# cwfparsonson/ddls

Hardware: NVIDIA H100
Metric: env_steps_per_sec (higher is better)
Workload: dtype f64

## Files before the change

ddls_b200/csrc/ramp_engine.cu:

```cuda
#include <algorithm>
#include <cmath>
#include <cstdio>
#include <cstdlib>
#include <cstring>
#include <map>
#include <mutex>
#include <numeric>
#include <utility>
#include <vector>

#include "ramp_kernels.cuh"
#include "ramp_env.cuh"
#include "ramp_owned.cuh"

using namespace ramp;

namespace {

constexpr int MAX_EVENT_PAIRS = 64;
constexpr int RAMP_SMEM_CARVEOUT = 100;

using LookaheadKernel = void (*)(const LookaheadArgs);
constexpr int WARP_NT = 128, SPLIT_WARP_NT = 32;
LookaheadKernel warp_kernel() { return ramp_lookahead_kernel<WARP_NT / 32>; }
// ... 16 lines not shown
}

using StepKernel = void (*)(const StepArgs);
constexpr size_t STEP_SMEM_MAX = 200 * 1024;
StepKernel step_kernel_for(int nt) { return nt == 32 ? ramp_step_kernel<32> : ramp_step_kernel<1>; }

struct HostTemplate {
    TemplateDev dev;
    DeviceArray<unsigned char> blob;
    std::vector<unsigned char> bytes;
    uint64_t hash = 0;
    DeviceArray<unsigned char> res_blob;
};

struct ResultArrays {
    DeviceArray<double> jct, comm, comp, util;
    DeviceArray<int32_t> n_ticks, status, util_nmw;
    DeviceArray<int64_t> trace_off;
    cudaError_t alloc(size_t n) { return alloc_each(n, jct, comm, comp, util, n_ticks, status, util_nmw, trace_off); }
    ResultSlots view() const { return {jct.get(), comm.get(), comp.get(), n_ticks.get(), status.get(), trace_off.get(), util.get(), util_nmw.get()}; }
};

struct TraceArrays {
    DeviceArray<int32_t> n_active;
    DeviceArray<double> tick;
    DeviceArray<unsigned long long> top;
    cudaError_t alloc(uint64_t len) {
        const cudaError_t err = alloc_each(len, n_active, tick);
        return err == cudaSuccess ? top.alloc(1) : err;
    }
    TracePool view() const { return TracePool{n_active.get(), tick.get(), top.get(), (uint64_t)n_active.size()}; }
};

constexpr int N_WINDOWS = 4;
struct LookaheadWindow {
    Stream stream;
    Event ev_planned, ev_end, ev_consumed;
    DeviceArray<Counters> counters;
    DeviceArray<WorkItem> items_res, chunk_items;
    DeviceArray<ChunkDesc> chunks;
    DeviceArray<int32_t> rank, tcount, tbase;
    DeviceArray<SpecRecord> rec;
    DeviceArray<unsigned char> scratch;
};

}

struct ramp_engine {
    ramp_config_t cfg{};
    int sm_count = 0;
    Stream stream;
    std::vector<HostTemplate> templates;
    DeviceArray<TemplateDev> d_templates;
    uint64_t max_scratch = 0;
    int32_t max_w = 1, max_c = 1;
    int32_t par_cap = 0;
    uint32_t memo_cap = 0;
    DeviceArray<unsigned long long> d_memo_keys;
    DeviceArray<int32_t> d_memo_vals;
    DeviceArray<unsigned long long> d_memo_keys2;
    uint32_t memo_cap2 = 0;
    ResultArrays res;
    int32_t n_slots = 0;
    TraceArrays pool;
    DeviceArray<WorkItem> d_items;
    DeviceArray<Counters> d_counters;
    DeviceArray<MemoStats> d_stats;
    DeviceArray<ramp_action_t> d_actions;
    DeviceArray<double> d_step_stats;
    DeviceArray<int32_t> d_n_cluster_steps;
    DeviceArray<double> d_ep_export;
    DeviceArray<double> d_es_export;
    EpisodeState ep{};
    DeviceArray<double> ep_ef, ep_es, ep_rf, tick_util; DeviceArray<int32_t> ep_ei, ep_ri, tick_util_n; DeviceArray<ramp_job_record_t> ep_rec;
    DeviceArray<ramp_arrival_t> d_arrivals;
    DeviceArray<int32_t> d_n_jobs_ep;
    PinnedArray<ramp_arrival_t> h_arr_stage;
    Event ev_stage;
    int step_nt = 0;
    size_t step_smem = 0;
    DeviceArray<unsigned char> d_scratch;
    uint64_t scratch_stride = 0;
    int grid = 0;
    size_t smem_bytes = 0;
    int cta_nt = 0;
    int dense_grid = 0;
    size_t dense_smem_bytes = 0;
    double dense_factor = 2.0;
    int cta_grid = 0;
    int cta64_grid = 0;
    int cta256_grid = 0;
    int cta_grid_for(int nt) const { return nt == 256 ? cta256_grid : nt == 128 ? cta_grid : cta64_grid; }
    size_t cta_smem_bytes = 0;
    size_t smem2_bytes = 0;
    int debug = 0;
    int mode = 0;
    PinnedArray<int32_t> h_n_work;
    PinnedArray<MemoStats> h_stats;
    DeviceArray<WorkItem> d_items_big;
    Stream stream2;
    Event ev_fork, ev_join;
    int use_quotient = 1;
    int n_resident = 0, n_nonresident = 0;
    int32_t res_tmpl_cap = 0, res_n_cap = 0, res_spill_ops = 0, res_spill_deps = 0;
    int res_grid = 0;
    size_t res_smem = 0;
    DeviceArray<unsigned char> d_res_scratch;
    uint64_t res_scratch_stride = 0;
    DeviceArray<WorkItem> d_items_res;
    DeviceArray<WorkItem> d_chunk_items;
    DeviceArray<ChunkDesc> d_chunks;
    DeviceArray<int32_t> d_tcount;
    DeviceArray<int32_t> d_tbase;
    DeviceArray<int32_t> d_rank;
    DeviceArray<TemplateHints> d_hints;
    DeviceArray<double> d_hint_jct;
    bool has_env = false;
    EnvDev env{};
    std::vector<DeviceArray<unsigned char>> env_allocs;
    PinnedArray<int32_t> env_h_need;
    PinnedArray<unsigned char> env_h_mirror;
    bool env_unchecked_decide = false;
    bool env_agents_set = false;
    DeviceArray<double> steplog_stats, steplog_rewards;
    DeviceArray<int32_t> steplog_actions;
    DeviceArray<WorkItem> sa_chunk_items;
    DeviceArray<ChunkDesc> sa_chunks;
    ResultArrays sa_res;
    int32_t sa_cap = 0;
    DeviceArray<WorkItem> sa_items;
    DeviceArray<int32_t> sa_rank;
    DeviceArray<Counters> sa_counters;
    int overlap = 1;
    LookaheadWindow win[N_WINDOWS];
    bool win_ready = false;
    uint64_t win_seq = 0;
    Stream plan_stream;
    Event ev_reset;
    bool reset_pending = false;
    DeviceArray<unsigned long long> d_spec_keys, d_repair_keys;
// ... 200 lines not shown
    if (!src.empty()) memcpy(blob.data() + h.off_src, src.data(), sizeof(int32_t) * src.size());
    return true;
}

int identity_quotient(const ramp_lowered_job_t* j, ramp_quotient_t* q) {
    memset(q, 0, sizeof(*q));
    const int32_t N = j->n_ops, E = j->n_deps;
    std::vector<uint32_t> ok, dk;
    make_rank_keys(j->op_prio, N, ok);
    make_rank_keys(j->dep_prio, E, dk);
    q->n_ops = N; q->n_deps = E; q->n_workers = j->n_workers; q->n_channels = j->n_channels;
    q->op_cost = (double*)malloc(sizeof(double) * N); q->op_key = (uint32_t*)malloc(4 * (size_t)N); q->op_worker = (uint32_t*)malloc(4 * (size_t)N);
    q->op_weight = (uint32_t*)malloc(4 * (size_t)N); q->op_threshold = (uint32_t*)malloc(4 * (size_t)N); q->row_ptr = (int32_t*)malloc(4 * ((size_t)N + 1));
    const size_t e1 = std::max(E, 1);
    q->dep_dst = (int32_t*)malloc(4 * e1); q->dep_run_time = (double*)malloc(8 * e1); q->dep_key = (uint32_t*)malloc(4 * e1);
    q->dep_channel = (uint32_t*)malloc(4 * e1); q->dep_is_flow = (uint8_t*)malloc(e1); q->dep_inc = (uint32_t*)malloc(4 * e1);
    q->dep_group_mask = (uint64_t*)malloc(8 * e1); q->merged = 0; q->masks_valid = j->n_channels <= 64 ? 1 : 0;
    q->op_class = (int32_t*)malloc(4 * (size_t)N); q->dep_entry = (int32_t*)malloc(4 * e1);
    for (int32_t i = 0; i < N; ++i) {
        q->op_cost[i] = j->op_cost[i]; q->op_key[i] = ok[i]; q->op_worker[i] = j->op_worker[i]; q->op_weight[i] = 1;
        q->op_threshold[i] = j->op_n_parents[i]; q->row_ptr[i] = j->row_ptr[i]; q->op_class[i] = i;
    }
    q->row_ptr[N] = j->row_ptr[N];
    for (int32_t k = 0; k < E; ++k) {
        q->dep_dst[k] = j->dep_dst[k]; q->dep_run_time[k] = j->dep_run_time[k]; q->dep_key[k] = dk[k];
        q->dep_channel[k] = (j->dep_channel[k] == RAMP_NO_CHANNEL) ? 0xFFFFFFFFu : (uint32_t)j->dep_channel[k];
        q->dep_group_mask[k] = (j->dep_channel[k] == RAMP_NO_CHANNEL || !q->masks_valid) ? 0ull : (1ull << j->dep_channel[k]);
        q->dep_is_flow[k] = j->dep_is_flow[k] ? 1 : 0; q->dep_inc[k] = 1; q->dep_entry[k] = k;
    }
    return RAMP_OK;
}

int ensure_thread_scratch(ramp_engine* e) {
    const size_t smem = thread_smem_bytes(e->res_tmpl_cap, e->res_n_cap);
    if (smem > 220 * 1024) return set_error(RAMP_ERR_CAPACITY, "resident templates need %zu B of shared memory (max 220 KiB)", smem);
    if (smem != e->res_smem || e->res_grid == 0) {
        CUDA_TRY(reserve_dynamic_smem((const void*)ramp_lookahead_thread_kernel, smem));
        CUDA_TRY(cudaFuncSetAttribute(ramp_lookahead_thread_kernel, cudaFuncAttributePreferredSharedMemoryCarveout, RAMP_SMEM_CARVEOUT));
        int occ = 0;
        CUDA_TRY(cudaOccupancyMaxActiveBlocksPerMultiprocessor(&occ, ramp_lookahead_thread_kernel, RAMP_THREAD_CTA, smem));
        if (occ < 1) occ = 1;
        const int want = (e->cfg.n_episodes + 31) / 32 + 8;
        e->res_grid = std::max(1, std::min(std::min(e->sm_count * occ, e->sm_count * 2), want));
        e->res_smem = smem;
        if (e->debug) fprintf(stderr, "[ramp] thread kernel: %zu B dynamic shared memory, %d CTAs of %d threads per SM fit, grid %d\n",
                              smem, occ, RAMP_THREAD_CTA, e->res_grid);
    }
    const uint64_t stride = thread_scratch_bytes(e->res_spill_ops, e->res_spill_deps, e->cfg.trace_cap);
    if (stride != e->res_scratch_stride || stride * (uint64_t)e->res_grid != e->d_res_scratch.size()) {
        CUDA_TRY(cudaStreamSynchronize(e->stream.get()));
        CUDA_TRY(e->d_res_scratch.alloc(stride * (uint64_t)e->res_grid));
        e->res_scratch_stride = stride;
    }
    return RAMP_OK;
}

ThreadArgs make_thread_args(ramp_engine* e, const ChunkDesc* chunks, const WorkItem* chunk_items, Counters* c,
                            const ResultSlots& res, const TracePool& pool, MemoStats* stats) {
    ThreadArgs a{};
    a.templates = e->d_templates.get(); a.chunks = chunks; a.n_chunks = &c->n_chunks; a.cursor = &c->chunk_cursor; a.items = chunk_items;
    a.scratch = e->d_res_scratch.get(); a.scratch_stride = e->res_scratch_stride;
    a.res = res; a.pool = pool; a.trace_cap = e->cfg.trace_cap;
    a.tmpl_cap = e->res_tmpl_cap; a.n_cap = e->res_n_cap; a.spill_ops = e->res_spill_ops; a.spill_deps = e->res_spill_deps;
    a.stats = stats; a.hints = e->d_hints.get(); a.hint_jct = e->d_hint_jct.get();
    return a;
}

void bucket_resident(ramp_engine* e, const WorkItem* items, Counters* c, WorkItem* chunk_items, ChunkDesc* chunks, int32_t* rank,
                     int32_t* tcount, int32_t* tbase, cudaStream_t st) {
    BucketArgs ba{};
    ba.items = items; ba.n_items = &c->n_work_res; ba.n_templates = (int32_t)e->templates.size();
    ba.tcount = tcount; ba.tbase = tbase; ba.chunk_items = chunk_items; ba.chunks = chunks;
    ba.n_chunks = &c->n_chunks; ba.cursor = &c->chunk_cursor; ba.rank = rank;
    ramp_bucket_kernel<<<1, 1024, 0, st>>>(ba);
    e->launches++;
}

int launch_lookaheads(ramp_engine* e, const ChunkDesc* chunks, const WorkItem* chunk_items, int thread_grid,
                      const WorkItem* items, int n_small, const WorkItem* items_big, int n_big, Counters* c,
                      const ResultSlots& res, const TracePool& pool, MemoStats* stats, cudaStream_t st) {
    if (thread_grid > 0) {
        ThreadArgs ta = make_thread_args(e, chunks, chunk_items, c, res, pool, stats);
        ramp_lookahead_thread_kernel<<<thread_grid, RAMP_THREAD_CTA, e->res_smem, st>>>(ta);
        e->launches++;
    }
    if (n_small + n_big == 0) return RAMP_OK;
    LookaheadArgs a = make_lookahead_args(e, items, c, res, pool, stats);
    LookaheadArgs ab = a;
    ab.items = items_big; ab.n_work = &c->n_work_big; ab.cursor = &c->work_cursor_big;
    const int wpb = WARP_NT / 32;
    const int warp_slots = e->grid * wpb;
    const int reg_slots = e->cta_grid * 4;
    int split_nt = 0;
    if (e->mode != 1 && n_big > 0) {
// ... 52 lines not shown
    if (src && n) CUDA_TRY(cudaMemcpy(e->env_allocs.back().get(), src, sizeof(T) * n, cudaMemcpyHostToDevice));
    else CUDA_TRY(cudaMemset(e->env_allocs.back().get(), 0, sizeof(T) * std::max<size_t>(n, 1)));
    return RAMP_OK;
}

bool engine_owned(const ramp_engine* e, const void* p) {
    const uintptr_t q = (uintptr_t)p;
    auto in = [q](const void* base, size_t bytes) { return q >= (uintptr_t)base && q < (uintptr_t)base + bytes; };
    if (in(e->d_actions.get(), sizeof(ramp_action_t) * e->d_actions.size())) return true;
    for (const auto& a : e->env_allocs) if (in(a.get(), a.size())) return true;
    return false;
}

int ensure_windows(ramp_engine* e) {
    const int B = e->cfg.n_episodes;
    const size_t nt = (size_t)e->cfg.max_templates + 1;
    if (!e->win_ready) {
        CUDA_TRY(create(e->plan_stream, cudaStreamNonBlocking));
        CUDA_TRY(create(e->ev_reset, cudaEventDisableTiming));
        for (LookaheadWindow& w : e->win) {
            CUDA_TRY(create(w.stream, cudaStreamNonBlocking));
            CUDA_TRY(create(w.ev_planned, cudaEventDisableTiming));
            CUDA_TRY(create(w.ev_end, cudaEventDisableTiming));
            CUDA_TRY(create(w.ev_consumed, cudaEventDisableTiming));
            CUDA_TRY(w.counters.alloc(1));
            CUDA_TRY(cudaMemset(w.counters.get(), 0, sizeof(Counters)));
            CUDA_TRY(alloc_each(B, w.items_res, w.chunks, w.rank, w.rec));
            CUDA_TRY(w.chunk_items.alloc((size_t)B * 32));
            CUDA_TRY(alloc_each(nt, w.tcount, w.tbase));
            CUDA_TRY(cudaMemset(w.tcount.get(), 0, sizeof(int32_t) * nt));
        }
        e->win_ready = true;
    }
    const uint64_t bytes = e->res_scratch_stride * (uint64_t)e->res_grid;
    for (LookaheadWindow& w : e->win) {
        if (w.scratch.size() == bytes) continue;
        CUDA_TRY(cudaStreamSynchronize(e->stream.get()));
        CUDA_TRY(w.scratch.alloc(bytes));
    }
    return RAMP_OK;
}

void launch_step_kernel(ramp_engine* e, const ramp_action_t* d_actions, int32_t fuse, double* d_stats_out, int32_t* d_ncs_out) {
    const int B = e->cfg.n_episodes;
    StepArgs s{};
    s.actions = d_actions; s.ep = e->ep; s.res = e->res.view(); s.pool = e->pool.view(); s.counters = e->d_counters.get();
    s.stats_out = d_stats_out; s.n_cluster_steps_out = d_ncs_out; s.fuse_empty_steps = fuse;
    step_kernel_for(e->step_nt)<<<(B + e->step_nt - 1) / e->step_nt, e->step_nt, e->step_smem, e->stream.get()>>>(s);
    e->launches++;
}

int step_overlapped(ramp_engine* e, const ramp_action_t* d_actions, int32_t fuse, double* d_stats_out, int32_t* d_ncs_out) {
    int rc = ensure_windows(e);
    if (rc != RAMP_OK) return rc;
    const int B = e->cfg.n_episodes, grid_b = (B + 127) / 128;
    const int32_t n_templates = (int32_t)e->templates.size();
    LookaheadWindow& w = e->win[e->win_seq++ % N_WINDOWS];
    cudaStream_t ps = e->plan_stream.get(), ws = w.stream.get(), st = e->stream.get();
    if (e->ev_pending >= MAX_EVENT_PAIRS) { CUDA_TRY(cudaStreamSynchronize(st)); rc = resolve_events(e); if (rc) return rc; }
    CUDA_TRY(cudaStreamWaitEvent(ps, w.ev_consumed.get(), 0));
    if (e->reset_pending) { CUDA_TRY(cudaStreamWaitEvent(ps, e->ev_reset.get(), 0)); e->reset_pending = false; }
    SpecPlanArgs sp{};
    sp.actions = d_actions; sp.templates = e->d_templates.get(); sp.n_templates = n_templates; sp.B = B;
    sp.keys = e->d_spec_keys.get(); sp.mask = e->memo_cap - 1; sp.slot_base = e->spec_base;
    sp.items_res = w.items_res.get(); sp.counters = w.counters.get(); sp.rec = w.rec.get();
    ramp_spec_plan_kernel<<<grid_b, 128, 0, ps>>>(sp);
    CUDA_TRY(cudaEventRecord(e->ev_a[e->ev_pending].get(), ps));
    bucket_resident(e, w.items_res.get(), w.counters.get(), w.chunk_items.get(), w.chunks.get(), w.rank.get(), w.tcount.get(), w.tbase.get(), ps);
    CUDA_TRY(cudaEventRecord(w.ev_planned.get(), ps));
    CUDA_TRY(cudaStreamWaitEvent(ws, w.ev_planned.get(), 0));
    ThreadArgs ta = make_thread_args(e, w.chunks.get(), w.chunk_items.get(), w.counters.get(), e->res.view(), e->pool.view(), e->d_stats.get());
    ta.scratch = w.scratch.get();
    ramp_lookahead_thread_kernel<<<e->res_grid, RAMP_THREAD_CTA, e->res_smem, ws>>>(ta);
    CUDA_TRY(cudaEventRecord(e->ev_b[e->ev_pending].get(), ws));
    e->ev_pending++;
    CUDA_TRY(cudaEventRecord(w.ev_end.get(), ws));
    CUDA_TRY(cudaStreamWaitEvent(st, w.ev_end.get(), 0));
    CommitArgs c{};
    c.actions = d_actions; c.templates = e->d_templates.get(); c.n_templates = n_templates; c.ep = e->ep;
    c.memo.keys = e->d_memo_keys.get(); c.memo.mask = e->memo_cap - 1; c.memo.mode = e->cfg.memo_mode; c.memo.vals = e->d_memo_vals.get();
    c.rec = w.rec.get(); c.repair_keys = e->d_repair_keys.get(); c.repair_mask = e->memo_cap - 1; c.repair_base = e->repair_base;
    c.items_res = w.items_res.get(); c.win_counters = w.counters.get(); c.counters = e->d_counters.get(); c.stats = e->d_stats.get();
    ramp_commit_kernel<<<grid_b, 128, 0, st>>>(c);
    bucket_resident(e, w.items_res.get(), w.counters.get(), w.chunk_items.get(), w.chunks.get(), w.rank.get(), w.tcount.get(), w.tbase.get(), st);
    ramp_lookahead_thread_kernel<<<e->res_grid, RAMP_THREAD_CTA, e->res_smem, st>>>(ta);
    launch_step_kernel(e, d_actions, fuse, d_stats_out, d_ncs_out);
    CUDA_TRY(cudaEventRecord(w.ev_consumed.get(), st));
    e->launches += 4;
    CUDA_TRY(cudaGetLastError());
    return RAMP_OK;
}

}

int ramp_internal_set_error(int code, const char* msg) { g_last_error = msg; return code; }
cudaStream_t ramp_internal_stream(ramp_engine_t* e) { return e->stream.get(); }
int ramp_internal_device(ramp_engine_t* e) { return e->cfg.device; }
void ramp_internal_count_launches(ramp_engine_t* e, int n) { e->launches += n; }
int ramp_internal_env_returns(ramp_engine_t* e, const double** ret, const int32_t** n_decided) {
    if (!e || !e->has_env) return set_error(RAMP_ERR_BAD_ARG, "no environment");
    *ret = e->env.ret;
    *n_decided = e->env.n_decided;
    return RAMP_OK;
}

extern "C" {

const char* ramp_last_error(void) { return g_last_error.c_str(); }

#ifdef RAMP_TICK_CLOCKS
int ramp_debug_tick_clocks(unsigned long long* out, int reset) {
    static unsigned long long h[RAMP_TC_MAX_CTAS][RAMP_TC_SHAPES][RAMP_TC_PHASES + 1];
    CUDA_TRY(cudaDeviceSynchronize());
    CUDA_TRY(cudaMemcpyFromSymbol(h, ramp::ramp_tick_clocks, sizeof(h)));
    memset(out, 0, sizeof(h[0]));
    for (int b = 0; b < RAMP_TC_MAX_CTAS; ++b)
        for (int s = 0; s < RAMP_TC_SHAPES; ++s)
            for (int i = 0; i <= RAMP_TC_PHASES; ++i) out[s * (RAMP_TC_PHASES + 1) + i] += h[b][s][i];
// ... 5 lines not shown
int ramp_engine_create(const ramp_config_t* cfg_in, ramp_engine_t** out) {
    if (!cfg_in || !out) return set_error(RAMP_ERR_BAD_ARG, "null argument");
    ramp_config_t cfg = *cfg_in;
    if (cfg.n_episodes < 1 || cfg.max_jobs < 1 || cfg.n_cluster_workers < 1)
        return set_error(RAMP_ERR_BAD_ARG, "n_episodes, max_jobs and n_cluster_workers must be >= 1");
    if (cfg.max_running < 1) cfg.max_running = cfg.n_cluster_workers;
    if (cfg.max_templates < 1) cfg.max_templates = 1024;
    if (cfg.trace_cap < 1) cfg.trace_cap = 16384;
    if (cfg.job_queue_capacity < 0) cfg.job_queue_capacity = 10;
    if (cfg.machine_epsilon == 0.0) cfg.machine_epsilon = 1e-7;
    if (cfg.memo_capacity_log2 <= 0) {
        int lg = 10;
        while ((1ll << lg) < (long long)cfg.n_episodes * 16 && lg < 26) ++lg;
        cfg.memo_capacity_log2 = lg;
    }
    CUDA_TRY(cudaSetDevice(cfg.device));
    std::unique_ptr<ramp_engine> e(new ramp_engine());
    e->cfg = cfg;
    if (const char* v = getenv("RAMP_LOOKAHEAD_CTA_THREADS")) {
        const int nt = atoi(v);
        if (lookahead_cta_kernel_for(nt) == nullptr) return set_error(RAMP_ERR_BAD_ARG, "RAMP_LOOKAHEAD_CTA_THREADS must be 64, 128 or 256");
        e->cta_nt = nt;
    }
    if (const char* v = getenv("RAMP_LOOKAHEAD_MODE")) {
        e->mode = !strcmp(v, "warp") ? 1 : !strcmp(v, "cta") ? 2 : 0;
        if (!strcmp(v, "thread_unfolded")) e->use_quotient = 0;
    }
    if (const char* v = getenv("RAMP_DEBUG")) e->debug = atoi(v);
    if (const char* v = getenv("RAMP_STEP_OVERLAP")) e->overlap = atoi(v) != 0;
    if (const char* v = getenv("RAMP_DENSE_FACTOR")) e->dense_factor = atof(v);
    cudaDeviceProp prop{};
    CUDA_TRY(cudaGetDeviceProperties(&prop, cfg.device));
    e->sm_count = prop.multiProcessorCount;
    CUDA_TRY(create(e->stream, cudaStreamNonBlocking));
    const int B = cfg.n_episodes;

    CUDA_TRY(e->d_templates.alloc(cfg.max_templates));
    e->memo_cap = 1u << cfg.memo_capacity_log2;
    CUDA_TRY(e->d_memo_keys.alloc(e->memo_cap));
    CUDA_TRY(cudaMemset(e->d_memo_keys.get(), 0, sizeof(unsigned long long) * e->memo_cap));
    CUDA_TRY(e->d_memo_vals.alloc(e->memo_cap));
    e->memo_cap2 = 1;
    while (e->memo_cap2 < (uint32_t)cfg.max_templates * 2u) e->memo_cap2 <<= 1;
    CUDA_TRY(e->d_memo_keys2.alloc(e->memo_cap2));
    CUDA_TRY(cudaMemset(e->d_memo_keys2.get(), 0, sizeof(unsigned long long) * e->memo_cap2));
    e->spec_base = (int32_t)e->memo_cap + B + (int32_t)e->memo_cap2;
    e->repair_base = e->spec_base + (int32_t)e->memo_cap;
    e->n_slots = e->repair_base + (int32_t)e->memo_cap;
    CUDA_TRY(alloc_each(e->memo_cap, e->d_spec_keys, e->d_repair_keys));
    CUDA_TRY(cudaMemset(e->d_spec_keys.get(), 0, sizeof(unsigned long long) * e->memo_cap));
    CUDA_TRY(cudaMemset(e->d_repair_keys.get(), 0, sizeof(unsigned long long) * e->memo_cap));
    CUDA_TRY(e->res.alloc(e->n_slots));
    CUDA_TRY(cudaMemset(e->res.status.get(), 0, sizeof(int32_t) * e->n_slots));

    CUDA_TRY(e->pool.alloc(std::max<uint64_t>(4ull << 20, (uint64_t)B * 8ull * 2048ull)));
    CUDA_TRY(cudaMemset(e->pool.top.get(), 0, sizeof(unsigned long long)));

    CUDA_TRY(alloc_each(B, e->d_items, e->d_items_big, e->d_items_res, e->d_chunks, e->d_rank, e->d_actions, e->d_n_cluster_steps));
    CUDA_TRY(e->d_chunk_items.alloc((size_t)B * 32));
    CUDA_TRY(alloc_each((size_t)cfg.max_templates + 1, e->d_tcount, e->d_tbase));
    CUDA_TRY(cudaMemset(e->d_tcount.get(), 0, sizeof(int32_t) * ((size_t)cfg.max_templates + 1)));
    CUDA_TRY(e->d_hints.alloc(cfg.max_templates));
    CUDA_TRY(cudaMemset(e->d_hints.get(), 0, sizeof(TemplateHints) * (size_t)cfg.max_templates));
    CUDA_TRY(e->d_hint_jct.alloc(cfg.max_templates));
    CUDA_TRY(cudaMemset(e->d_hint_jct.get(), 0, sizeof(double) * (size_t)cfg.max_templates));
    CUDA_TRY(create(e->stream2, cudaStreamNonBlocking));
    CUDA_TRY(create(e->ev_fork, cudaEventDisableTiming));
// ... 148 lines not shown

    CUDA_TRY(cudaSetDevice(e->cfg.device));
    CUDA_TRY(ht.blob.alloc(total));
    CUDA_TRY(cudaMemcpy(ht.blob.get(), ht.bytes.data(), total, cudaMemcpyHostToDevice));
    unsigned char* base = ht.blob.get();
    TemplateDev& d = ht.dev;
    d.n_ops = N; d.n_deps = E; d.n_workers = W; d.n_channels = C;
    d.num_training_steps = j->num_training_steps; d.model_id = j->model_id; d.degree = j->degree;
    d.n_src = (int32_t)src.size(); d.canon_id = canon;
    d.size_class = ((int64_t)N + (int64_t)E >= BIG_THRESHOLD) ? 1 : 0;
    d.par_in_smem = par_in_smem ? 1 : 0;
    d._pad0 = 0;
    d.op_rec = (const int4*)(base + segs[0].off); d.op_n_parents = (const uint16_t*)(base + segs[1].off);
    d.op_row = (const int2*)(base + segs[2].off); d.dep_kd = (const unsigned long long*)(base + segs[3].off);
    d.dep_rt = (const double*)(base + segs[4].off); d.src_ops = (const int32_t*)(base + segs[5].off);
    d.kd_kmask = kd_kmask; d.kd_cmask = kd_cmask; d.kd_cshift = kd_cshift; d.kd_fshift = kd_fshift; d.kd_dshift = kd_dshift; d._pad1 = 0;
    d.scratch_bytes = scratch_bytes_for(N, E);
    d.algorithmic_bytes_static = 20ull * (uint64_t)N + 19ull * (uint64_t)E + 24ull;
    d.res_blob = nullptr; d.res_bytes = 0; d.res_n_ops = 0; d.res_n_deps = 0; d._pad2 = 0;
    if (e->mode == 0) {
        ramp_quotient_t q{};
        const int qrc = e->use_quotient ? ramp_quotient_template(j, &q) : identity_quotient(j, &q);
        if (qrc != RAMP_OK) return set_error(qrc, "ramp_quotient_template failed (%d)", qrc);
        std::vector<unsigned char> rblob;
        if (build_resident_blob(j, q, RESIDENT_MAX_BYTES, rblob)) {
            cudaError_t ce = ht.res_blob.alloc(rblob.size());
            if (ce == cudaSuccess) ce = cudaMemcpy(ht.res_blob.get(), rblob.data(), rblob.size(), cudaMemcpyHostToDevice);
            if (ce != cudaSuccess) { ramp_free_quotient(&q); return set_error(RAMP_ERR_CUDA, "resident blob upload failed: %s", cudaGetErrorString(ce)); }
            d.res_blob = ht.res_blob.get(); d.res_bytes = (int32_t)rblob.size();
            d.res_n_ops = q.n_ops; d.res_n_deps = q.n_deps;
            d.size_class = 2;
            e->res_tmpl_cap = std::max(e->res_tmpl_cap, (int32_t)align_up((uint64_t)rblob.size(), 128));
            e->res_n_cap = std::max(e->res_n_cap, (int32_t)align_up((uint64_t)q.n_ops, 2));
            e->res_spill_ops = std::max(e->res_spill_ops, q.n_ops);
            e->res_spill_deps = std::max(e->res_spill_deps, std::max(q.n_deps, 1));
        }
        if (e->debug) fprintf(stderr, "[ramp] template %d: N=%d E=%d W=%d C=%d -> quotient N=%d E=%d W=%d C=%d, %s (%zu B)\n", (int)e->templates.size(),
                              N, E, W, C, q.n_ops, q.n_deps, q.n_workers, q.n_channels, d.res_blob ? "resident" : "not resident", rblob.size());
        ramp_free_quotient(&q);
    }
    const int32_t id = (int32_t)e->templates.size();
    CUDA_TRY(cudaMemcpy(e->d_templates.get() + id, &d, sizeof(TemplateDev), cudaMemcpyHostToDevice));
    if (d.size_class == 2) e->n_resident++; else e->n_nonresident++;
    if (d.size_class != 2) {
        e->max_scratch = std::max(e->max_scratch, d.scratch_bytes);
        e->max_w = std::max(e->max_w, W);
        e->max_c = std::max(e->max_c, std::max(C, 1));
        if (d.par_in_smem) e->par_cap = std::max(e->par_cap, (int32_t)align_up((uint64_t)N, 16));
    }
    e->templates.push_back(std::move(ht));
    *id_out = id;
    return RAMP_OK;
}

int ramp_reset(ramp_engine_t* e, const ramp_arrival_t* arrivals, int32_t n_jobs) {
    if (!e || !arrivals) return set_error(RAMP_ERR_BAD_ARG, "null argument");
    if (n_jobs < 1 || n_jobs > e->cfg.max_jobs) return set_error(RAMP_ERR_BAD_ARG, "n_jobs %d not in [1, max_jobs=%d]", n_jobs, e->cfg.max_jobs);
    CUDA_TRY(cudaSetDevice(e->cfg.device));
    const int B = e->cfg.n_episodes;
    cudaStream_t st = e->stream.get();
    CUDA_TRY(cudaEventSynchronize(e->ev_stage.get()));
    const size_t row = sizeof(ramp_arrival_t) * (size_t)n_jobs;
    memcpy(e->h_arr_stage.get(), arrivals, row * B);
    if (n_jobs == e->cfg.max_jobs) {
        CUDA_TRY(cudaMemcpyAsync(e->d_arrivals.get(), e->h_arr_stage.get(), row * B, cudaMemcpyHostToDevice, st));
    } else {
// ... 733 lines not shown
```

ddls_b200/csrc/ramp_lookahead_thread.cuh:

```cuda
#pragma once

namespace ramp {

#ifndef RAMP_T_OCAP
#define RAMP_T_OCAP 8
#endif
#ifndef RAMP_T_FCAP
#define RAMP_T_FCAP 16
#endif
#ifndef RAMP_T_FASTF
#define RAMP_T_FASTF 6
#endif
#ifndef RAMP_T_NFCAP
#define RAMP_T_NFCAP 8
#endif
#define RAMP_T_WCAP 8
#define RAMP_T_CCAP 32
#ifndef RAMP_T_RING
#define RAMP_T_RING 32
#endif
#ifndef RAMP_T_PUB
#define RAMP_T_PUB 8
#endif
static_assert(RAMP_T_FCAP >= RAMP_T_FASTF && RAMP_T_OCAP >= 2 && RAMP_T_NFCAP >= 1, "shared-memory capacities below the small-frontier path");
#define RAMP_T_DONE 0x80000000u
#define RAMP_THREAD_CTA 64

struct ResHeader {
    int32_t n_ops, n_deps, n_workers, n_channels;
    int32_t n_src, num_training_steps, orig_workers, _pad0;
    uint32_t kmask, cmask, imask, _pad1;
    int32_t cshift, fshift, ishift, dshift;
    int32_t off_op_row, off_op_thr, off_out, off_src;
    int32_t total_bytes, _pad2, _pad3, _pad4;
};
static_assert(sizeof(ResHeader) == 96, "resident header is 96 bytes");

struct ChunkDesc { int32_t template_id, count; };
static_assert((RAMP_T_RING & (RAMP_T_RING - 1)) == 0 && (RAMP_T_PUB & (RAMP_T_PUB - 1)) == 0 && RAMP_T_PUB <= RAMP_T_RING,
              "ring and publish interval are powers of two");

struct __align__(16) TemplateHints { int32_t n_ticks, max_o, max_f, max_nf; };


struct ThreadArgs {
    const TemplateDev* templates;
    const ChunkDesc* chunks;
    const int32_t* n_chunks;
    int32_t* cursor;
    const WorkItem* items;
    unsigned char* scratch;
    uint64_t scratch_stride;
    ResultSlots res;
    TracePool pool;
    int32_t trace_cap;
    int32_t tmpl_cap;
    int32_t n_cap;
    int32_t spill_ops, spill_deps;
    MemoStats* stats;
    TemplateHints* hints;
    double* hint_jct;
};

__host__ __device__ inline size_t thread_smem_bytes(int tmpl_cap, int n_cap) {
    size_t per_lane = (size_t)RAMP_T_RING * 16 + (size_t)RAMP_T_FCAP * 16 + (size_t)RAMP_T_OCAP * 20 + (size_t)RAMP_T_NFCAP * 4
                      + (size_t)(RAMP_T_WCAP + RAMP_T_CCAP) * 4 + (size_t)n_cap * 2;
    return (size_t)tmpl_cap + 32 * per_lane + 64;
}
__host__ __device__ inline uint64_t thread_scratch_bytes(int spill_ops, int spill_deps, int trace_cap) {
    const uint64_t per_lane = (uint64_t)spill_ops * 20 + (uint64_t)spill_deps * 20 + (uint64_t)trace_cap * 12;
    return align_up(per_lane * 32, 256);
}

struct BucketArgs {
    const WorkItem* items;
    int32_t* n_items;
    int32_t n_templates;
    int32_t* tcount;
    int32_t* tbase;
    WorkItem* chunk_items;
    ChunkDesc* chunks;
    int32_t* n_chunks;
    int32_t* cursor;
    int32_t* rank;
};

__global__ void __launch_bounds__(1024) ramp_bucket_kernel(const BucketArgs a) {
    __shared__ int s_scan[1024];
    __shared__ int s_carry;
    const int n = *a.n_items;
    const int tid = threadIdx.x;
    for (int i = tid; i < n; i += blockDim.x) a.rank[i] = atomicAdd(&a.tcount[a.items[i].template_id], 1);
    if (tid == 0) s_carry = 0;
    __syncthreads();
    for (int base = 0; base < a.n_templates; base += blockDim.x) {
        const int t = base + tid;
        const int cnt = (t < a.n_templates) ? a.tcount[t] : 0;
        const int nch = (cnt + 31) >> 5;
        s_scan[tid] = nch;
// ... 463 lines not shown
        for (; k != end; ++k) {
            const int4 r = y.ring[(k & (RAMP_T_RING - 1)) * 32 + y.lane];
            const u64_t tick_b = rem_bits(r);
            const double tick = __longlong_as_double((long long)tick_b);
            const int n_active = r.z;
            if (r.w) S.comm = __dadd_rn(S.comm, tick);
            if (n_active > 0) {
                S.comp = __dadd_rn(S.comp, tick);
                if (do_util && tick_b != 0ull) {
                    if (n_active != util_last_n) { util_last_n = n_active; util_last_q = __ddiv_rn((double)n_active, y.util_dn); }
                    S.util = __dadd_rn(S.util, __dmul_rn(util_last_q, __ddiv_rn(tick, y.util_jct)));
                }
            }
            S.t = __dadd_rn(S.t, tick);
            if ((int)k < y.tr_cap) { y.tr_n[tr_idx] = n_active; y.tr_tick[tr_idx] = tick; tr_idx += y.tr_stride; }
#ifdef RAMP_T_LEDGER_NS
            __nanosleep(RAMP_T_LEDGER_NS);
#endif
        }
        st_release_cta(y.tail, k);
    }
    return S;
}

__global__ void __launch_bounds__(RAMP_THREAD_CTA) ramp_lookahead_thread_kernel(const ThreadArgs a) {
    extern __shared__ __align__(128) unsigned char smem_thr[];
    __shared__ __align__(8) unsigned long long mbar;
    __shared__ uint32_t s_head[32], s_tail[32];
    __shared__ SimFinal s_fin[32];
    __shared__ int32_t s_tr_cap[32];
    __shared__ int4 s_chunk;
    __shared__ int4 s_hint;
    __shared__ double s_hint_jct;
    const int lane = threadIdx.x & 31;
    const bool is_sim = threadIdx.x < 32;
    unsigned char* st = smem_thr + a.tmpl_cap;
    int4* ring = reinterpret_cast<int4*>(st);
    LaneCtx x;
    x.tm = smem_thr;
    x.f_sm = ring + RAMP_T_RING * 32;
    x.o_sm = x.f_sm + RAMP_T_FCAP * 32;
    x.nf_sm = reinterpret_cast<uint32_t*>(x.o_sm + RAMP_T_OCAP * 32);
    x.oi_sm = reinterpret_cast<int32_t*>(x.nf_sm + RAMP_T_NFCAP * 32);
    x.wk_sm = reinterpret_cast<uint32_t*>(x.oi_sm + RAMP_T_OCAP * 32);
    x.ck_sm = x.wk_sm + RAMP_T_WCAP * 32;
    x.cnt_sm = reinterpret_cast<uint16_t*>(x.ck_sm + RAMP_T_CCAP * 32);
    unsigned char* slab = a.scratch + (uint64_t)blockIdx.x * a.scratch_stride;
    x.f_gl = reinterpret_cast<int4*>(slab);
    x.o_gl = x.f_gl + (size_t)a.spill_deps * 32;
    double* tmp_tick = reinterpret_cast<double*>(x.o_gl + (size_t)a.spill_ops * 32);
    x.nf_gl = reinterpret_cast<uint32_t*>(tmp_tick + (size_t)a.trace_cap * 32);
    x.oi_gl = reinterpret_cast<int32_t*>(x.nf_gl + (size_t)a.spill_deps * 32);
    int32_t* tmp_n = x.oi_gl + (size_t)a.spill_ops * 32;
    x.ring = ring; x.head = &s_head[lane]; x.tail = &s_tail[lane]; x.fin = &s_fin[lane];
    x.lane = lane; x.n_cap = a.n_cap;

    if (threadIdx.x == 0) {
        asm volatile("mbarrier.init.shared::cta.b64 [%0], 1;" ::"r"(smem_u32(&mbar)));
        asm volatile("fence.mbarrier_init.release.cluster;" ::: "memory");
    }
    __syncthreads();
    uint32_t phase = 0;
    int loaded = -1;

    for (;;) {
        asm volatile("fence.proxy.async.shared::cta;" ::: "memory");
        if (threadIdx.x == 0) {
            int4 cd = make_int4(0, -1, 0, 0), hv = make_int4(0, 0, 0, 0);
            double hj = 0.0;
            const int c = atomicAdd(a.cursor, 1);
            if (c < *a.n_chunks) {
                const ChunkDesc ch = a.chunks[c];
                cd = make_int4(c, ch.template_id, ch.count, 0);
                const TemplateHints* hp = &a.hints[ch.template_id];
                int n_ticks = 0;
                asm volatile("ld.acquire.gpu.global.b32 %0, [%1];" : "=r"(n_ticks) : "l"(&hp->n_ticks) : "memory");
                if (n_ticks > 0) {
                    hv = make_int4(n_ticks, __ldcg(&hp->max_o), __ldcg(&hp->max_f), __ldcg(&hp->max_nf));
                    hj = __ldcg(&a.hint_jct[ch.template_id]);
                }
            }
            s_chunk = cd; s_hint = hv; s_hint_jct = hj;
        }
        __syncthreads();
        const int4 cd = s_chunk;
        if (cd.y < 0) break;
        const int c = cd.x, tmpl = cd.y, count = cd.z;
        TemplateHints hint;
        { const int4 hv = s_hint; hint.n_ticks = hv.x; hint.max_o = hv.y; hint.max_f = hv.z; hint.max_nf = hv.w; }
        const double hj = s_hint_jct;
        const TemplateDev& TD = a.templates[tmpl];
        if (tmpl != loaded) {
            if (threadIdx.x == 0) {
                const uint32_t bytes = (uint32_t)TD.res_bytes;
                asm volatile("mbarrier.arrive.expect_tx.shared::cta.b64 _, [%0], %1;" ::"r"(smem_u32(&mbar)), "r"(bytes) : "memory");
                asm volatile("cp.async.bulk.shared::cluster.global.mbarrier::complete_tx::bytes [%0], [%1], %2, [%3];"
                             ::"r"(smem_u32(smem_thr)), "l"(TD.res_blob), "r"(bytes), "r"(smem_u32(&mbar)) : "memory");
            }
            asm volatile(
                "{\n"
                ".reg .pred p;\n"
                "RAMP_WAIT_%=:\n"
                "mbarrier.try_wait.parity.shared::cta.b64 p, [%0], %1;\n"
                "@p bra RAMP_DONE_%=;\n"
                "bra RAMP_WAIT_%=;\n"
                "RAMP_DONE_%=:\n"
                "}\n" ::"r"(smem_u32(&mbar)), "r"(phase) : "memory");
            phase ^= 1u;
            loaded = tmpl;
        }
        const bool fast = hint.n_ticks > 0 && hint.n_ticks <= a.trace_cap && hint.max_o <= RAMP_T_OCAP && hint.max_f <= RAMP_T_FCAP
                          && hint.max_nf <= RAMP_T_NFCAP;
        const ResHeader& H = *reinterpret_cast<const ResHeader*>(x.tm);
        const bool active = lane < count;

        LedgerCtx y;
        WorkItem item;
        long long off = -1;
        int status0 = RAMP_ST_OK, nmw = 0, num_training_steps = 0, n_ops = 0, n_deps = 0;
        const bool direct = fast && a.pool.top != nullptr;
        if (!is_sim) {
            s_head[lane] = 0u; s_tail[lane] = 0u;
            if (active) {
                item = a.items[(size_t)c * 32 + lane];
                num_training_steps = H.num_training_steps; n_ops = H.n_ops; n_deps = H.n_deps;
                if (direct) {
                    const unsigned long long o = atomicAdd(a.pool.top, (unsigned long long)hint.n_ticks);
                    if (o + (unsigned long long)hint.n_ticks <= a.pool.len) off = (long long)o; else status0 = RAMP_ST_TRACE_OVERFLOW;
                }
                y.ring = ring; y.head = &s_head[lane]; y.tail = &s_tail[lane]; y.lane = lane;
                if (off >= 0) { y.tr_n = a.pool.n_active + off; y.tr_tick = a.pool.tick + off; y.tr_stride = 1; y.tr_cap = hint.n_ticks; }
                else { y.tr_n = tmp_n + lane; y.tr_tick = tmp_tick + lane; y.tr_stride = 32; y.tr_cap = a.trace_cap; }
                s_tr_cap[lane] = y.tr_cap;
                nmw = item.n_mounted_workers > 0 ? item.n_mounted_workers : H.orig_workers;
                y.util_jct = (fast && hj > 0.0 && !isinf(hj)) ? hj : 0.0;
                {
                    double dn = (double)nmw;
                    asm volatile("" : "+d"(dn));
                    y.util_dn = dn;
                }
            }
        }
        __syncthreads();

        if (is_sim) {
            if (active) {
                x.tr_cap = s_tr_cap[lane];
                if (fast) thread_lookahead<false>(x);
                else thread_lookahead<true>(x);
            }
            continue;
        }
        if (!active) continue;
        const LedgerSums S = ledger_run(y);
        const SimFinal R = s_fin[lane];
        int status = (R.status == RAMP_ST_OK) ? status0 : R.status;
        if (direct && status == RAMP_ST_OK && R.tick_no != hint.n_ticks) status = RAMP_ST_TRACE_OVERFLOW;
        if (!fast && status == RAMP_ST_OK) {
            TemplateHints* hp = &a.hints[tmpl];
            hp->max_o = R.max_o; hp->max_f = R.max_f; hp->max_nf = R.max_nf;
            a.hint_jct[tmpl] = __dmul_rn(S.t, (double)num_training_steps);
            asm volatile("st.release.gpu.global.b32 [%0], %1;" :: "l"(&hp->n_ticks), "r"(R.tick_no) : "memory");
        }

        const int n_rec = R.tick_no < y.tr_cap ? R.tick_no : y.tr_cap;
        const double steps = (double)num_training_steps;
        const double jct = __dmul_rn(S.t, steps);
        const bool can_util = (status == RAMP_ST_OK);
        const bool util_done = can_util && y.util_jct != 0.0 && jct == y.util_jct;
        if (!direct && a.pool.top != nullptr) {
            const unsigned long long o = atomicAdd(a.pool.top, (unsigned long long)n_rec);
            if (o + (unsigned long long)n_rec <= a.pool.len) off = (long long)o;
            else if (status == RAMP_ST_OK) status = RAMP_ST_TRACE_OVERFLOW;
        }
        double util = util_done ? S.util : 0.0;
        if (!(util_done && (direct || off < 0))) {
            if (util_done) util = 0.0;
            const double dn = (double)nmw;
            const bool copy = (!direct) && off >= 0;
            int32_t* pn = copy ? a.pool.n_active + off : nullptr;
            double* pt = copy ? a.pool.tick + off : nullptr;
            const int32_t* sn = y.tr_n; const double* stt = y.tr_tick; const int sstr = y.tr_stride;
            const bool skip_zero = can_util && (jct > 0.0) && !isinf(jct);
            int last_n = -1;
            double last_q = 0.0;
#pragma unroll 4
            for (int k = 0; k < n_rec; ++k) {
                const int nk = sn[(size_t)k * sstr];
                const double tk = stt[(size_t)k * sstr];
                if (copy) { pn[k] = nk; pt[k] = tk; }
                if (!can_util) continue;
                if (skip_zero && (nk == 0 || tk == 0.0)) continue;
                if (nk != last_n) { last_n = nk; last_q = __ddiv_rn((double)nk, dn); }
                util = __dadd_rn(util, __dmul_rn(last_q, __ddiv_rn(tk, jct)));
            }
        }
        a.res.jct[item.slot] = jct;
        a.res.comm[item.slot] = __dmul_rn(S.comm, steps);
        a.res.comp[item.slot] = __dmul_rn(S.comp, steps);
        a.res.n_ticks[item.slot] = R.tick_no;
        a.res.util[item.slot] = can_util ? util : 0.0;
        a.res.util_nmw[item.slot] = can_util ? nmw : -1;
        a.res.trace_off[item.slot] = off;
        a.res.status[item.slot] = status;
        if (a.stats) {
            atomicAdd(&a.stats->lookaheads, 1ull);
            atomicAdd(&a.stats->alg_bytes, (unsigned long long)(TD.algorithmic_bytes_static + 12ull * (unsigned long long)R.tick_no));
            atomicAdd(&a.stats->quotient_bytes, (unsigned long long)(20ull * n_ops + 19ull * n_deps + 24ull + 12ull * (unsigned long long)R.tick_no));
        }
    }
}

}
```

ddls_b200/csrc/ramp_owned.cuh:

```cuda
#pragma once

#include <atomic>
#include <cstdarg>
#include <cstdio>
#include <memory>
#include <string>

#include <cuda_runtime.h>

#include "../../include/ramp_b200.h"

namespace ramp {

#pragma GCC visibility push(hidden)
inline thread_local std::string g_last_error;

inline int set_error(int code, const char* fmt, ...) {
    char buf[1024];
    va_list ap;
    va_start(ap, fmt);
    vsnprintf(buf, sizeof(buf), fmt, ap);
    va_end(ap);
    g_last_error = buf;
    return code;
// ... 34 lines not shown
        (Pinned ? g_pinned_bytes : g_device_bytes) += (int64_t)bytes;
        return cudaSuccess;
    }
    T* get() const { return p_.get(); }
    size_t size() const { return p_ ? p_.get_deleter().bytes / sizeof(T) : 0; }
private:
    std::unique_ptr<T, ArrayFree<Pinned>> p_;
};

template <class T> using DeviceArray = OwnedArray<T, false>;
template <class T> using PinnedArray = OwnedArray<T, true>;

template <class... Arrays> cudaError_t alloc_each(size_t n, Arrays&... arrays) {
    cudaError_t err = cudaSuccess;
    ((err = (err == cudaSuccess ? arrays.alloc(n) : err)), ...);
    return err;
}

struct CudaDestroy {
    void operator()(cudaStream_t s) const { cudaStreamDestroy(s); }
    void operator()(cudaEvent_t ev) const { cudaEventDestroy(ev); }
};
using Stream = std::unique_ptr<CUstream_st, CudaDestroy>;
using Event = std::unique_ptr<CUevent_st, CudaDestroy>;
inline cudaError_t create_raw(cudaStream_t* s, unsigned flags) { return cudaStreamCreateWithFlags(s, flags); }
inline cudaError_t create_raw(cudaEvent_t* ev, unsigned flags) { return cudaEventCreateWithFlags(ev, flags); }

template <class Owner> cudaError_t create(Owner& o, unsigned flags) {
    typename Owner::pointer raw = nullptr;
    const cudaError_t err = create_raw(&raw, flags);
    o.reset(raw);
    return err;
}

}
```

Baseline: 13.16 million.

## Share spill scratch via slot leasing, widen windows, shrink repair grid, prioritize stream

Per-window spill scratch buffers are replaced by one shared pool of slabs. CTAs lease a slab with atomicCAS only when they take the slow (spilling) path, which cuts scratch memory and lets more lookahead windows run (8 instead of 4). Shared memory for channel keys is now sized to the real maximum channel count instead of a fixed cap, which may raise occupancy. The repair lookahead launch is capped at a few CTAs, and the main stream is created at the highest priority. The trade-off is spin-wait contention on slots across concurrent windows and possible serialization when many CTAs spill at once.

Measured after the change: 14.97 million (median of 6 runs). 13.8% higher.

```diff
diff --git a/ddls_b200/csrc/ramp_engine.cu b/ddls_b200/csrc/ramp_engine.cu
--- a/ddls_b200/csrc/ramp_engine.cu
+++ b/ddls_b200/csrc/ramp_engine.cu
@@ -72,7 +72,8 @@
     TracePool view() const { return TracePool{n_active.get(), tick.get(), top.get(), (uint64_t)n_active.size()}; }
 };
 
-constexpr int N_WINDOWS = 4;
+constexpr int N_WINDOWS = 8;
+constexpr int REPAIR_GRID = 4;
 struct LookaheadWindow {
     Stream stream;
     Event ev_planned, ev_end, ev_consumed;
@@ -81,7 +82,6 @@
     DeviceArray<ChunkDesc> chunks;
     DeviceArray<int32_t> rank, tcount, tbase;
     DeviceArray<SpecRecord> rec;
-    DeviceArray<unsigned char> scratch;
 };
 
 }
@@ -142,10 +142,12 @@
     Event ev_fork, ev_join;
     int use_quotient = 1;
     int n_resident = 0, n_nonresident = 0;
-    int32_t res_tmpl_cap = 0, res_n_cap = 0, res_spill_ops = 0, res_spill_deps = 0;
+    int32_t res_tmpl_cap = 0, res_n_cap = 0, res_c_cap = 0, res_spill_ops = 0, res_spill_deps = 0;
     int res_grid = 0;
+    int res_occ = 0;
     size_t res_smem = 0;
     DeviceArray<unsigned char> d_res_scratch;
+    DeviceArray<int32_t> d_res_slot_busy;
     uint64_t res_scratch_stride = 0;
     DeviceArray<WorkItem> d_items_res;
     DeviceArray<WorkItem> d_chunk_items;
@@ -412,7 +414,7 @@
 }
 
 int ensure_thread_scratch(ramp_engine* e) {
-    const size_t smem = thread_smem_bytes(e->res_tmpl_cap, e->res_n_cap);
+    const size_t smem = thread_smem_bytes(e->res_tmpl_cap, e->res_n_cap, std::max(e->res_c_cap, 1));
     if (smem > 220 * 1024) return set_error(RAMP_ERR_CAPACITY, "resident templates need %zu B of shared memory (max 220 KiB)", smem);
     if (smem != e->res_smem || e->res_grid == 0) {
         CUDA_TRY(reserve_dynamic_smem((const void*)ramp_lookahead_thread_kernel, smem));
@@ -422,14 +424,19 @@
         if (occ < 1) occ = 1;
         const int want = (e->cfg.n_episodes + 31) / 32 + 8;
         e->res_grid = std::max(1, std::min(std::min(e->sm_count * occ, e->sm_count * 2), want));
+        e->res_occ = occ;
         e->res_smem = smem;
         if (e->debug) fprintf(stderr, "[ramp] thread kernel: %zu B dynamic shared memory, %d CTAs of %d threads per SM fit, grid %d\n",
                               smem, occ, RAMP_THREAD_CTA, e->res_grid);
     }
     const uint64_t stride = thread_scratch_bytes(e->res_spill_ops, e->res_spill_deps, e->cfg.trace_cap);
-    if (stride != e->res_scratch_stride || stride * (uint64_t)e->res_grid != e->d_res_scratch.size()) {
+    if (stride != e->res_scratch_stride || stride * (uint64_t)e->res_grid != e->d_res_scratch.size()
+        || (size_t)e->res_grid != e->d_res_slot_busy.size()) {
         CUDA_TRY(cudaStreamSynchronize(e->stream.get()));
         CUDA_TRY(e->d_res_scratch.alloc(stride * (uint64_t)e->res_grid));
+        CUDA_TRY(e->d_res_slot_busy.alloc(e->res_grid));
+        CUDA_TRY(cudaMemsetAsync(e->d_res_slot_busy.get(), 0, sizeof(int32_t) * e->res_grid, e->stream.get()));
+        CUDA_TRY(cudaStreamSynchronize(e->stream.get()));
         e->res_scratch_stride = stride;
     }
     return RAMP_OK;
@@ -440,6 +447,8 @@
     ThreadArgs a{};
     a.templates = e->d_templates.get(); a.chunks = chunks; a.n_chunks = &c->n_chunks; a.cursor = &c->chunk_cursor; a.items = chunk_items;
     a.scratch = e->d_res_scratch.get(); a.scratch_stride = e->res_scratch_stride;
+    a.slot_busy = e->d_res_slot_busy.get(); a.n_slots = e->res_grid; a.slots_per_sm = std::max(1, e->res_grid / e->sm_count);
+    a.c_cap = std::max(e->res_c_cap, 1);
     a.res = res; a.pool = pool; a.trace_cap = e->cfg.trace_cap;
     a.tmpl_cap = e->res_tmpl_cap; a.n_cap = e->res_n_cap; a.spill_ops = e->res_spill_ops; a.spill_deps = e->res_spill_deps;
     a.stats = stats; a.hints = e->d_hints.get(); a.hint_jct = e->d_hint_jct.get();
@@ -558,12 +567,6 @@
         }
         e->win_ready = true;
     }
-    const uint64_t bytes = e->res_scratch_stride * (uint64_t)e->res_grid;
-    for (LookaheadWindow& w : e->win) {
-        if (w.scratch.size() == bytes) continue;
-        CUDA_TRY(cudaStreamSynchronize(e->stream.get()));
-        CUDA_TRY(w.scratch.alloc(bytes));
-    }
     return RAMP_OK;
 }
 
@@ -596,7 +599,6 @@
     CUDA_TRY(cudaEventRecord(w.ev_planned.get(), ps));
     CUDA_TRY(cudaStreamWaitEvent(ws, w.ev_planned.get(), 0));
     ThreadArgs ta = make_thread_args(e, w.chunks.get(), w.chunk_items.get(), w.counters.get(), e->res.view(), e->pool.view(), e->d_stats.get());
-    ta.scratch = w.scratch.get();
     ramp_lookahead_thread_kernel<<<e->res_grid, RAMP_THREAD_CTA, e->res_smem, ws>>>(ta);
     CUDA_TRY(cudaEventRecord(e->ev_b[e->ev_pending].get(), ws));
     e->ev_pending++;
@@ -609,7 +611,7 @@
     c.items_res = w.items_res.get(); c.win_counters = w.counters.get(); c.counters = e->d_counters.get(); c.stats = e->d_stats.get();
     ramp_commit_kernel<<<grid_b, 128, 0, st>>>(c);
     bucket_resident(e, w.items_res.get(), w.counters.get(), w.chunk_items.get(), w.chunks.get(), w.rank.get(), w.tcount.get(), w.tbase.get(), st);
-    ramp_lookahead_thread_kernel<<<e->res_grid, RAMP_THREAD_CTA, e->res_smem, st>>>(ta);
+    ramp_lookahead_thread_kernel<<<std::min(e->res_grid, REPAIR_GRID), RAMP_THREAD_CTA, e->res_smem, st>>>(ta);
     launch_step_kernel(e, d_actions, fuse, d_stats_out, d_ncs_out);
     CUDA_TRY(cudaEventRecord(w.ev_consumed.get(), st));
     e->launches += 4;
@@ -681,7 +683,11 @@
     cudaDeviceProp prop{};
     CUDA_TRY(cudaGetDeviceProperties(&prop, cfg.device));
     e->sm_count = prop.multiProcessorCount;
-    CUDA_TRY(create(e->stream, cudaStreamNonBlocking));
+    {
+        int least = 0, greatest = 0;
+        CUDA_TRY(cudaDeviceGetStreamPriorityRange(&least, &greatest));
+        CUDA_TRY(create(e->stream, cudaStreamNonBlocking, greatest));
+    }
     const int B = cfg.n_episodes;
 
     CUDA_TRY(e->d_templates.alloc(cfg.max_templates));
@@ -896,6 +902,7 @@
             d.size_class = 2;
             e->res_tmpl_cap = std::max(e->res_tmpl_cap, (int32_t)align_up((uint64_t)rblob.size(), 128));
             e->res_n_cap = std::max(e->res_n_cap, (int32_t)align_up((uint64_t)q.n_ops, 2));
+            e->res_c_cap = std::max(e->res_c_cap, std::max(q.n_channels, 1));
             e->res_spill_ops = std::max(e->res_spill_ops, q.n_ops);
             e->res_spill_deps = std::max(e->res_spill_deps, std::max(q.n_deps, 1));
         }
diff --git a/ddls_b200/csrc/ramp_lookahead_thread.cuh b/ddls_b200/csrc/ramp_lookahead_thread.cuh
--- a/ddls_b200/csrc/ramp_lookahead_thread.cuh
+++ b/ddls_b200/csrc/ramp_lookahead_thread.cuh
@@ -51,6 +51,9 @@
     const WorkItem* items;
     unsigned char* scratch;
     uint64_t scratch_stride;
+    int32_t* slot_busy;
+    int32_t n_slots, slots_per_sm;
+    int32_t c_cap;
     ResultSlots res;
     TracePool pool;
     int32_t trace_cap;
@@ -62,9 +65,9 @@
     double* hint_jct;
 };
 
-__host__ __device__ inline size_t thread_smem_bytes(int tmpl_cap, int n_cap) {
+__host__ __device__ inline size_t thread_smem_bytes(int tmpl_cap, int n_cap, int c_cap) {
     size_t per_lane = (size_t)RAMP_T_RING * 16 + (size_t)RAMP_T_FCAP * 16 + (size_t)RAMP_T_OCAP * 20 + (size_t)RAMP_T_NFCAP * 4
-                      + (size_t)(RAMP_T_WCAP + RAMP_T_CCAP) * 4 + (size_t)n_cap * 2;
+                      + (size_t)(RAMP_T_WCAP + c_cap) * 4 + (size_t)n_cap * 2;
     return (size_t)tmpl_cap + 32 * per_lane + 64;
 }
 __host__ __device__ inline uint64_t thread_scratch_bytes(int spill_ops, int spill_deps, int trace_cap) {
@@ -594,6 +597,7 @@
     __shared__ int4 s_chunk;
     __shared__ int4 s_hint;
     __shared__ double s_hint_jct;
+    __shared__ int32_t s_slot;
     const int lane = threadIdx.x & 31;
     const bool is_sim = threadIdx.x < 32;
     unsigned char* st = smem_thr + a.tmpl_cap;
@@ -606,14 +610,7 @@
     x.oi_sm = reinterpret_cast<int32_t*>(x.nf_sm + RAMP_T_NFCAP * 32);
     x.wk_sm = reinterpret_cast<uint32_t*>(x.oi_sm + RAMP_T_OCAP * 32);
     x.ck_sm = x.wk_sm + RAMP_T_WCAP * 32;
-    x.cnt_sm = reinterpret_cast<uint16_t*>(x.ck_sm + RAMP_T_CCAP * 32);
-    unsigned char* slab = a.scratch + (uint64_t)blockIdx.x * a.scratch_stride;
-    x.f_gl = reinterpret_cast<int4*>(slab);
-    x.o_gl = x.f_gl + (size_t)a.spill_deps * 32;
-    double* tmp_tick = reinterpret_cast<double*>(x.o_gl + (size_t)a.spill_ops * 32);
-    x.nf_gl = reinterpret_cast<uint32_t*>(tmp_tick + (size_t)a.trace_cap * 32);
-    x.oi_gl = reinterpret_cast<int32_t*>(x.nf_gl + (size_t)a.spill_deps * 32);
-    int32_t* tmp_n = x.oi_gl + (size_t)a.spill_ops * 32;
+    x.cnt_sm = reinterpret_cast<uint16_t*>(x.ck_sm + (size_t)a.c_cap * 32);
     x.ring = ring; x.head = &s_head[lane]; x.tail = &s_tail[lane]; x.fin = &s_fin[lane];
     x.lane = lane; x.n_cap = a.n_cap;
 
@@ -624,6 +621,7 @@
     __syncthreads();
     uint32_t phase = 0;
     int loaded = -1;
+    int held = -1;
 
     for (;;) {
         asm volatile("fence.proxy.async.shared::cta;" ::: "memory");
@@ -675,12 +673,31 @@
                           && hint.max_nf <= RAMP_T_NFCAP;
         const ResHeader& H = *reinterpret_cast<const ResHeader*>(x.tm);
         const bool active = lane < count;
+        const bool direct = fast && a.pool.top != nullptr;
+        if (threadIdx.x == 0) {
+            if (direct && held >= 0) { __threadfence(); atomicExch(&a.slot_busy[held], 0); held = -1; }
+            if (!direct && held < 0) {
+                uint32_t smid;
+                asm volatile("mov.u32 %0, %%smid;" : "=r"(smid));
+                int q = (int)((smid * (uint32_t)a.slots_per_sm) % (uint32_t)a.n_slots);
+                while (atomicCAS(&a.slot_busy[q], 0, 1) != 0) { q = (q + 1 == a.n_slots) ? 0 : q + 1; __nanosleep(256); }
+                __threadfence();
+                held = q;
+            }
+            s_slot = held;
+        }
+        __syncthreads();
+        auto slab = [&]() { return a.scratch + (uint64_t)s_slot * a.scratch_stride; };
+        auto tmp_tick = [&]() { return reinterpret_cast<double*>(slab() + ((size_t)a.spill_deps + a.spill_ops) * 32 * 16); };
+        auto tmp_n = [&]() {
+            return reinterpret_cast<int32_t*>(slab() + ((size_t)a.spill_deps + a.spill_ops) * 32 * 16 + (size_t)a.trace_cap * 32 * 8
+                                              + ((size_t)a.spill_deps + a.spill_ops) * 32 * 4);
+        };
 
         LedgerCtx y;
         WorkItem item;
         long long off = -1;
         int status0 = RAMP_ST_OK, nmw = 0, num_training_steps = 0, n_ops = 0, n_deps = 0;
-        const bool direct = fast && a.pool.top != nullptr;
         if (!is_sim) {
             s_head[lane] = 0u; s_tail[lane] = 0u;
             if (active) {
@@ -692,7 +709,7 @@
                 }
                 y.ring = ring; y.head = &s_head[lane]; y.tail = &s_tail[lane]; y.lane = lane;
                 if (off >= 0) { y.tr_n = a.pool.n_active + off; y.tr_tick = a.pool.tick + off; y.tr_stride = 1; y.tr_cap = hint.n_ticks; }
-                else { y.tr_n = tmp_n + lane; y.tr_tick = tmp_tick + lane; y.tr_stride = 32; y.tr_cap = a.trace_cap; }
+                else { y.tr_n = tmp_n() + lane; y.tr_tick = tmp_tick() + lane; y.tr_stride = 32; y.tr_cap = a.trace_cap; }
                 s_tr_cap[lane] = y.tr_cap;
                 nmw = item.n_mounted_workers > 0 ? item.n_mounted_workers : H.orig_workers;
                 y.util_jct = (fast && hj > 0.0 && !isinf(hj)) ? hj : 0.0;
@@ -709,7 +726,13 @@
             if (active) {
                 x.tr_cap = s_tr_cap[lane];
                 if (fast) thread_lookahead<false>(x);
-                else thread_lookahead<true>(x);
+                else {
+                    x.f_gl = reinterpret_cast<int4*>(slab());
+                    x.o_gl = x.f_gl + (size_t)a.spill_deps * 32;
+                    x.nf_gl = reinterpret_cast<uint32_t*>(tmp_tick() + (size_t)a.trace_cap * 32);
+                    x.oi_gl = reinterpret_cast<int32_t*>(x.nf_gl + (size_t)a.spill_deps * 32);
+                    thread_lookahead<true>(x);
+                }
             }
             continue;
         }
@@ -771,6 +794,7 @@
             atomicAdd(&a.stats->quotient_bytes, (unsigned long long)(20ull * n_ops + 19ull * n_deps + 24ull + 12ull * (unsigned long long)R.tick_no));
         }
     }
+    if (threadIdx.x == 0 && held >= 0) { __threadfence(); atomicExch(&a.slot_busy[held], 0); }
 }
 
 }
diff --git a/ddls_b200/csrc/ramp_owned.cuh b/ddls_b200/csrc/ramp_owned.cuh
--- a/ddls_b200/csrc/ramp_owned.cuh
+++ b/ddls_b200/csrc/ramp_owned.cuh
@@ -90,5 +90,11 @@
     o.reset(raw);
     return err;
 }
+inline cudaError_t create(Stream& o, unsigned flags, int priority) {
+    cudaStream_t raw = nullptr;
+    const cudaError_t err = cudaStreamCreateWithPriority(&raw, flags, priority);
+    o.reset(raw);
+    return err;
+}
 
 }
```
